# linyueqian/HippoMM

Hardware: AMD Instinct MI355X
Metric: frame-embeddings/sec (ImageBind-huge ViT-H/14 vision tower; scan GB/s under 'scan') (higher is better)
Workload: dtype bf16; 1 GPU; BASELINE cfg2: ViT-H/14 vision encoder (32 blocks, 257 tokens, D=1280), 256 synthetic 224x224 frames per GPU per step (scenes of 6 frames), random-init weights; step = encode -> (N>1: RCCL all-gather of embeddings) -> cosine key-frame selection; frames_per_gpu=256, kept_key_frames=9, of_frames=256

## Files before the change

### hippomm_amd/_lib.py

```python
from __future__ import annotations

import ctypes as C
from pathlib import Path

_PKG = Path(__file__).resolve().parent
LIB_PATH = _PKG / "libhippomm_hip.so"

_lib = None

c_f32p = C.c_void_p
c_ptr = C.c_void_p

_SIGNATURES = {
    "hmm_abi_version": (C.c_int, []),
    "hmm_last_error": (C.c_char_p, []),
    "hmm_device_supported": (C.c_int, []),
    "hmm_cosine_topk_workspace_bytes": (C.c_size_t, [C.c_int64, C.c_int]),
    "hmm_cosine_topk": (C.c_int, [c_ptr, C.c_int64, C.c_int, c_ptr, C.c_int, c_ptr, c_ptr, c_ptr,
                                  c_ptr, C.c_size_t, c_ptr]),
    "hmm_cosine_topk_keys": (C.c_int, [c_ptr, C.c_int64, C.c_int, c_ptr, C.c_int, c_ptr,
                                       c_ptr, C.c_size_t, c_ptr]),
    "hmm_topk_merge_keys": (C.c_int, [c_ptr, C.c_int, C.c_int, c_ptr, c_ptr, c_ptr, c_ptr, c_ptr]),
    "hmm_shadow_store_bytes": (C.c_size_t, [C.c_int64]),
    "hmm_shadow_store_build": (C.c_int, [c_ptr, C.c_int64, C.c_int, c_ptr, C.c_size_t, c_ptr]),
# ... 67 lines not shown
    "hmm_jpeg_workspace_bytes": (C.c_size_t, [c_ptr, C.c_int, C.c_int, C.c_int, C.c_int, C.c_int]),
    "hmm_jpeg_reconstruct": (C.c_int, [c_ptr, C.c_int, C.c_size_t, c_ptr, C.c_int, C.c_int, C.c_int, C.c_int, c_ptr, c_ptr,
                                       C.c_size_t, c_ptr]),
    "hmm_jpeg_entropy_slot_bytes": (C.c_int64, [C.c_size_t]),
    "hmm_jpeg_prepare_entropy": (C.c_int, [c_ptr, C.c_size_t, c_ptr, c_ptr, C.c_size_t]),
    "hmm_jpeg_entropy_workspace_bytes": (C.c_size_t, [c_ptr, C.c_int, C.c_size_t]),
    "hmm_jpeg_decode_coefs_device": (C.c_int, [c_ptr, C.c_int, C.c_size_t, c_ptr, C.c_int, C.c_int, C.c_int, C.c_int, c_ptr,
                                               C.c_size_t, c_ptr, c_ptr, C.c_size_t, c_ptr]),
    "hmm_jpeg_encode_header": (C.c_int, [c_ptr, C.c_int, c_ptr, C.c_size_t, c_ptr]),
    "hmm_jpeg_encode_workspace_bytes": (C.c_size_t, [c_ptr, C.c_int]),
    "hmm_jpeg_encode_bound": (C.c_size_t, [c_ptr]),
    "hmm_jpeg_encode": (C.c_int, [c_ptr, C.c_int, c_ptr, C.c_int, C.c_int, c_ptr, c_ptr, C.c_size_t, c_ptr, C.c_size_t, c_ptr,
                                  c_ptr, C.c_size_t, c_ptr]),
    "hmm_jpeg_encoded_pixels_workspace_bytes": (C.c_size_t, [c_ptr, C.c_int, C.c_int, C.c_int, C.c_int, C.c_int]),
    "hmm_jpeg_encoded_pixels": (C.c_int, [c_ptr, C.c_int, c_ptr, c_ptr, C.c_int, C.c_int, C.c_int, C.c_int, c_ptr, c_ptr,
                                          C.c_size_t, c_ptr]),
    "hmm_encoder_create":(C.c_int, [C.POINTER(C.c_void_p), C.c_int, C.c_int]),
    "hmm_encoder_destroy": (None, [c_ptr]),
    "hmm_encoder_load_param": (C.c_int, [c_ptr, C.c_char_p, c_ptr, C.c_int64, c_ptr]),
    "hmm_encoder_missing_params": (C.c_int, [c_ptr]),
    "hmm_encoder_workspace_bytes": (C.c_size_t, [c_ptr, C.c_int]),
    "hmm_encoder_forward": (C.c_int, [c_ptr, c_ptr, C.c_int, c_ptr, c_ptr, C.c_size_t, c_ptr]),
    "hmm_encoder_flops": (C.c_double, [c_ptr, C.c_int]),
    "hmm_encoder_flops_executed": (C.c_double, [c_ptr, C.c_int]),
    "hmm_encoder_set_streams": (C.c_int, [c_ptr, C.c_int]),
    "hmm_encoder_set_fused_attention": (C.c_int, [c_ptr, C.c_int]),
    "hmm_encoder_text_packed_workspace_bytes": (C.c_size_t, [c_ptr, C.c_int, C.c_int64]),
    "hmm_encoder_forward_text_packed": (C.c_int, [c_ptr, c_ptr, c_ptr, c_ptr, C.c_int, c_ptr, c_ptr, C.c_size_t, c_ptr]),
    "hmm_op_attention_causal_packed_bf16": (C.c_int, [c_ptr, c_ptr, c_ptr, C.c_int, C.c_int, C.c_int, C.c_int, c_ptr]),
    "hmm_op_gemm_bf16": (C.c_int, [c_ptr, c_ptr, c_ptr, c_ptr, C.c_int, C.c_int, C.c_int, C.c_int, c_ptr]),
    "hmm_op_layernorm_bf16": (C.c_int, [c_ptr, c_ptr, c_ptr, c_ptr, C.c_int, C.c_int, C.c_float, c_ptr]),
    "hmm_op_gemm_bf16_tile": (C.c_int, [c_ptr, c_ptr, c_ptr, c_ptr, C.c_int, C.c_int, C.c_int, C.c_int, C.c_int, c_ptr]),
    "hmm_op_gemm_bf16_splitk": (C.c_int, [c_ptr, c_ptr, c_ptr, C.c_int, C.c_int, C.c_int, C.c_int, C.c_int, c_ptr]),
    "hmm_op_gemm_plan": (C.c_int, [C.c_int, C.c_int, C.c_int, C.c_int, C.c_int, C.c_int, C.c_int, c_ptr, C.c_int]),
    "hmm_op_layernorm_reduce_bf16": (C.c_int, [c_ptr, c_ptr, C.c_int, c_ptr, c_ptr, c_ptr, c_ptr, C.c_int, C.c_int, C.c_float, c_ptr]),
    "hmm_op_attention_bf16": (C.c_int, [c_ptr, c_ptr, C.c_int, C.c_int, C.c_int, C.c_int, c_ptr, c_ptr, c_ptr]),
    "hmm_op_qkv_attention_bf16": (C.c_int, [c_ptr, c_ptr, c_ptr, c_ptr, c_ptr, C.c_int, c_ptr]),
    "hmm_op_qkv_attention_audio_bf16": (C.c_int, [c_ptr, c_ptr, c_ptr, c_ptr, c_ptr, c_ptr, C.c_int, c_ptr]),
    "hmm_op_attention_causal_bf16": (C.c_int, [c_ptr, c_ptr, C.c_int, C.c_int, C.c_int, C.c_int, c_ptr]),
    "hmm_op_im2col_vision_bf16": (C.c_int, [c_ptr, c_ptr, C.c_int, c_ptr]),
    "hmm_op_im2col_audio_bf16": (C.c_int, [c_ptr, c_ptr, C.c_int, c_ptr]),
    "hmm_op_fold_conv3d_bf16": (C.c_int, [c_ptr, c_ptr, C.c_int, c_ptr]),
    "hmm_op_assemble_tokens": (C.c_int, [c_ptr, c_ptr, c_ptr, c_ptr, c_ptr, C.c_float, c_ptr, c_ptr, C.c_float, c_ptr,
                                         C.c_int, C.c_int, C.c_int, c_ptr]),
    "hmm_op_layernorm_strided_bf16": (C.c_int, [c_ptr, C.c_size_t, c_ptr, c_ptr, c_ptr, C.c_int, C.c_int, C.c_float, c_ptr]),
    "hmm_op_gather_rows": (C.c_int, [c_ptr, C.c_size_t, c_ptr, C.c_int, C.c_int, c_ptr]),
    "hmm_op_attention_cls_bf16": (C.c_int, [c_ptr, c_ptr, c_ptr, C.c_int, C.c_int, C.c_int, C.c_int, c_ptr, c_ptr, c_ptr]),
    "hmm_op_embed_tokens": (C.c_int, [c_ptr, c_ptr, c_ptr, c_ptr, C.c_int, C.c_int, C.c_int, c_ptr]),
    "hmm_op_layernorm_eos_bf16": (C.c_int, [c_ptr, c_ptr, C.c_int, c_ptr, c_ptr, c_ptr, C.c_int, C.c_int, C.c_float, c_ptr]),
    "hmm_op_l2norm_rows": (C.c_int, [c_ptr, c_ptr, C.c_int, C.c_int, c_ptr, c_ptr]),
    "hmm_op_scan_topk_only": (C.c_int, [c_ptr, C.c_int64, c_ptr, C.c_int, c_ptr, c_ptr]),
    "hmm_op_scan_sims": (C.c_int, [c_ptr, C.c_int64, c_ptr, c_ptr, c_ptr]),
    "hmm_json_find_matrices": (C.c_int, [C.c_char_p, C.c_size_t, C.c_size_t, c_ptr, C.c_int, C.POINTER(C.c_int)]),
    "hmm_json_parse_matrix_f32": (C.c_int, [C.c_char_p, C.c_size_t, C.c_size_t, C.c_size_t, C.c_size_t, c_ptr]),
    "hmm_json_matrix_text_bound": (C.c_size_t, [C.c_size_t, C.c_size_t, C.c_int]),
    "hmm_json_write_matrix_f64": (C.c_int, [c_ptr, C.c_size_t, C.c_size_t, C.c_int, c_ptr, C.c_size_t, C.POINTER(C.c_size_t)]),
    "hmm_json_write_matrix_device_workspace_bytes": (C.c_size_t, [C.c_size_t, C.c_size_t]),
    "hmm_json_write_matrix_device": (C.c_int, [c_ptr, C.c_int, C.c_size_t, C.c_size_t, C.c_int, c_ptr, C.c_size_t, c_ptr, c_ptr,
                                               C.c_size_t, c_ptr]),
    "hmm_json_float_repr": (C.c_int, [c_ptr, C.c_size_t, c_ptr, c_ptr]),
    "hmm_json_parse_matrix_device_workspace_bytes": (C.c_size_t, [C.c_size_t]),
    "hmm_json_parse_matrix_device": (C.c_int, [c_ptr, C.c_size_t, C.c_size_t, C.c_size_t, C.c_size_t, C.c_int, c_ptr, c_ptr, c_ptr,
                                               C.c_int64, c_ptr, C.c_size_t, c_ptr]),
    "hmm_json_float_parse": (C.c_int, [c_ptr, c_ptr, C.c_size_t, c_ptr, c_ptr, c_ptr]),
    "hmm_json_find_matrices_device_workspace_bytes": (C.c_size_t, [C.c_size_t]),
    "hmm_json_find_matrices_device": (C.c_int, [c_ptr, C.c_size_t, C.c_size_t, c_ptr, C.c_int, c_ptr, c_ptr, C.c_size_t, c_ptr]),
    "hmm_json_find_matrices_blocks": (C.c_int, [c_ptr, C.c_size_t, C.c_size_t, c_ptr, C.c_int, c_ptr]),
    "hmm_base64_encoded_length": (C.c_size_t, [C.c_size_t]),
    "hmm_base64_encode_device": (C.c_int, [c_ptr, C.c_int, C.c_size_t, c_ptr, C.c_size_t, c_ptr]),
    "hmm_base64_decode_device": (C.c_int, [c_ptr, C.c_size_t, C.c_int, c_ptr, C.c_size_t, c_ptr, c_ptr]),
    "hmm_base64_encode_host": (C.c_int, [c_ptr, C.c_int, C.c_size_t, c_ptr, C.c_size_t]),
# ... 54 lines not shown
```

### hippomm_amd/csrc/gemm_bf16.hip

```cpp
#include <string>
#include <type_traits>
#include "hmm_common.h"
#include "encoder_ops.h"
#include "gemm_pp_mainloop.h"

namespace hmm {

__device__ __forceinline__ float gelu_erf(float x) {
    const float u = fabsf(x);
    const float t = __builtin_amdgcn_rcpf(fmaf(0.3275911f * 0.70710678118654752440f, u, 1.0f));
    float poly = fmaf(t, 0.5f * 1.061405429f, 0.5f * -1.453152027f);
    poly = fmaf(poly, t, 0.5f * 1.421413741f);
    poly = fmaf(poly, t, 0.5f * -0.284496736f);
    poly = fmaf(poly, t, 0.5f * 0.254829592f);
    poly *= t;
    const float e = __builtin_amdgcn_exp2f(u * u * (-0.5f * 1.4426950408889634f));
    return fmaxf(x, 0.0f) - u * poly * e;
}

template <int EPI, int MI, int NI>
__device__ __forceinline__ void gemm_epilogue(f32x4 (&acc)[MI][NI], const float* __restrict__ bias,
                                              void* __restrict__ Cout, int M, int N, int m_lane, int n_lane) {
    float4 bv[NI];
#pragma unroll
    for (int ni = 0; ni < NI; ++ni)
        bv[ni] = bias ? *reinterpret_cast<const float4*>(bias + n_lane + ni * 16) : make_float4(0.f, 0.f, 0.f, 0.f);

    if constexpr (EPI == HMM_EPI_BIAS_RESID_F32) {
        float* C = static_cast<float*>(Cout);
        float4 xin[2][NI];
        auto load_row = [&](int mi, float4 (&dst)[NI]) {
            const int m = m_lane + mi * 16;
            if (m < M) {
#pragma unroll
                for (int ni = 0; ni < NI; ++ni)
                    dst[ni] = *reinterpret_cast<const float4*>(C + (size_t)m * N + n_lane + ni * 16);
            }
// ... 352 lines not shown
            }
        };
        auto slab_free = [&]() {
            asm volatile("s_waitcnt lgkmcnt(0)" ::: "memory");
            __builtin_amdgcn_wave_barrier();
        };
        if constexpr (RESID) { load_resid(0, 0); load_resid(0, 1); }
        park(0);
        drain(0);
        drain(1);
        slab_free();
        park(1);
        drain(2);
        drain(3);
    }
}

template <int EPI>
__device__ __forceinline__ void gemm_epilogue_lds(f32x4 (&acc)[8][4], const float* __restrict__ bias,
                                                  void* __restrict__ Cout, int M, int N, int m_wave, int n_wave,
                                                  char* slab, int lane) {
    const int fq = lane >> 4;
    float4 bv[4];
#pragma unroll
    for (int ni = 0; ni < 4; ++ni)
        bv[ni] = bias ? *reinterpret_cast<const float4*>(bias + n_wave + ni * 16 + 4 * fq) : make_float4(0.f, 0.f, 0.f, 0.f);
    if (m_wave + 128 <= M)
        gemm_epilogue_lds_body<EPI, false>(acc, bv, Cout, M, N, m_wave, n_wave, slab, lane);
    else if (m_wave < M)
        gemm_epilogue_lds_body<EPI, true>(acc, bv, Cout, M, N, m_wave, n_wave, slab, lane);
}

HMM_TUNABLE(int, g_gemm_walk, -1)
static int pick_walk(int tiles_m, int tiles_n) {
    if (g_gemm_walk >= 0) return g_gemm_walk;
    return (tiles_n >= 10 && tiles_n % 5 == 0 && tiles_m >= 48) ? ((6 << 8) | 5) : 0;
}

template <int EPI>
__global__ __launch_bounds__(512) void gemm_bf16_pp_kernel(
    const bf16_t* __restrict__ A, const bf16_t* __restrict__ W, const float* __restrict__ bias,
    void* __restrict__ Cout, int M, int N, int K, int tiles_n, int walk) {
    extern __shared__ __attribute__((aligned(16))) char smem[];

    const int lane = threadIdx.x & 63;
    const int wave = __builtin_amdgcn_readfirstlane(threadIdx.x >> 6);
    const int wm = wave >> 2, wn = wave & 3;

    const int nb = gridDim.x, bid = blockIdx.x;
    const int q8 = nb >> 3, r8 = nb & 7, xcd = bid & 7;
    const int swz = (xcd < r8 ? xcd * (q8 + 1) : r8 * (q8 + 1) + (xcd - r8) * q8) + (bid >> 3);
    int m0 = (swz / tiles_n) * 256, n0 = (swz % tiles_n) * 256;
    if (walk) {
        const int R = walk >> 8, C = walk & 255, tiles_m = nb / tiles_n;
        const int rg = swz / (R * tiles_n), rem = swz - rg * R * tiles_n;
        const int rows_g = tiles_m - R * rg < R ? tiles_m - R * rg : R;
        const int cg = rem / (rows_g * C), rem2 = rem - cg * rows_g * C;
        const int wc = tiles_n - C * cg < C ? tiles_n - C * cg : C;
        m0 = (rg * R + rem2 / wc) * 256;
        n0 = (cg * C + rem2 % wc) * 256;
    }

    PPSources src;
#pragma unroll
    for (int j = 0; j < 2; ++j) {
        const int lr = (wave + 8 * j) * 8 + (lane >> 3);
        const int c = (lane & 7) ^ ((lr >> 1) & 7);
        const int arow = (lr & 63) + (lr >> 6) * 128;
        int g0 = m0 + arow, g1 = m0 + arow + 64;
        g0 = g0 < M ? g0 : M - 1;
        g1 = g1 < M ? g1 : M - 1;
        src.alo[j] = g0 * K + c * 8;
        src.ahi[j] = g1 * K + c * 8;
        const int bcol = (lr >> 5) * 64 + (lr & 31);
        src.blo[j] = (n0 + bcol) * K + c * 8;
        src.bhi[j] = (n0 + bcol + 32) * K + c * 8;
    }

    f32x4 acc[8][4];
#pragma unroll
    for (int mi = 0; mi < 8; ++mi)
#pragma unroll
        for (int ni = 0; ni < 4; ++ni) acc[mi][ni] = f32x4{0.f, 0.f, 0.f, 0.f};

    pp_mainloop(A, W, src, K >> 6, smem, lane, wave, acc);

    int lane_e = lane;
    asm volatile("" : "+v"(lane_e));
    gemm_epilogue_lds<EPI>(acc, bias, Cout, M, N, m0 + wm * 128, n0 + wn * 64, smem + wave * kEpiSlab, lane_e);
}

template <int EPI>
static int launch_gemm_pp(const bf16_t* A, const bf16_t* W, const float* bias, void* C, int M, int N, int K,
                          hipStream_t st) {
    constexpr int LDS = 8 * kEpiSlab > 2 * 4 * 16384 ? 8 * kEpiSlab : 2 * 4 * 16384;
    const int tiles_m = (M + 255) / 256, tiles_n = N / 256;
    auto kern = gemm_bf16_pp_kernel<EPI>;
    HMM_ENSURE_DYN_LDS(kern, LDS);
    kern<<<tiles_m * tiles_n, 512, LDS, st>>>(A, W, bias, C, M, N, K, tiles_n, pick_walk(tiles_m, tiles_n));
    HMM_LAUNCH_CHECK();
    return HMM_OK;
}

template <int BM, int BN, int WM, int WN, int EPI, int STAGES, int KSUB>
static int launch_gemm(const bf16_t* A, const bf16_t* W, const float* bias, void* C, int M, int N, int K, int splits,
                       hipStream_t st) {
    constexpr int LDS = STAGES * KSUB * (BM + BN) * 128;
    static_assert(LDS <= 160 * 1024, "ring of the tiled GEMM: LDS");
    auto kern = gemm_bf16_kernel<BM, BN, WM, WN, EPI, STAGES, KSUB>;
    HMM_ENSURE_DYN_LDS(kern, LDS);
    const int tiles_m = (M + BM - 1) / BM, tiles_n = N / BN;
    kern<<<tiles_m * tiles_n * splits, WM * WN * 64, LDS, st>>>(A, W, bias, C, M, N, K, tiles_n, tiles_m, K / splits);
    HMM_LAUNCH_CHECK();
    return HMM_OK;
}

struct DispatchRule { const char* knob; int limit; int off; const char* what; const char* forwards; const char* evidence; };
constexpr DispatchRule kDispatchRules[] = {
    {"g_gemm_small_64", 512, 0, "launches of at most this many 64x64 tiles run on them behind the 4-deep ring (else 128x128 ring / double buffer)",
     "text:1,4;vision:1,2;audio:1", "r3_sliver_probe.json, r3_text_latency.json"},
    {"g_gemm_small_32", 400, 0, "launches of at most this many 32x32 tiles run on them (one 16x16 block per wave)",
     "text:1,2;vision:1", "r3_text_latency.json"},
    {"g_gemm_deepk", 1, 0, "deep-K rings: 2 / 4 K-tiles per stage while most CUs have a workgroup of their own (32x32: <= 192 / 256 tiles, 64x64: <= 256)",
     "text:1,2;vision:1", "r4_deepk_probe.json"},
    {"g_gemm_ring8", 1, 0, "the 128-row ring tiles (128x128, 128x64) with eight waves instead of four",
     "vision:1,8;audio:1;text:9", "r5_rect_tile_probe2.json, r5_ring8_ab.json"},
    {"g_gemm_rect", 1, 0, "128x64 ring tiles when 64x64 tiles outnumber the CUs but 128x64 tiles do not, up to g_gemm_rect_rows rows",
     "vision:1;text:4,6;audio:1", "r5_rect_tile_probe.json, r5_rect_forward2.json"},
    {"g_gemm_rect_rows", 700, 320, "row limit of the 128x64 rule (320 = the four-wave tile's)",
     "text:5,6,7,8;audio:1", "r5_rect700_ab.json"},
    {"g_gemm_rect_rows_longk", 1536, 0, "the 128x64 rule's row limit for K >= 5120 (fc2 of three to five frames)",
     "vision:3,4,5", "r5_rect_longk_ab.json"},
// ... 267 lines not shown
    HMM_REQUIRE(M >= 1 && N >= 128 && N % 128 == 0 && splits >= 1 && splits <= 8 && K % (64 * splits) == 0, HMM_E_INVALID,
                "gemm_splitk: unsupported shape M=%d N=%d K=%d splits=%d", M, N, K, splits);
    if (tile < 0) {
        const long w64 = (long)((M + 63) / 64) * (N / 64) * splits;
        const bool k2 = (K / splits) % 128 == 0;
        if (w64 <= 128) tile = k2 ? HMM_GEMM_TILE_32x32_RING_K2 : HMM_GEMM_TILE_32x32_RING;
        else if (w64 <= 256) tile = k2 ? HMM_GEMM_TILE_64x64_RING_K2 : HMM_GEMM_TILE_64x64_RING;
        else if (w64 > 448 && (long)((M + 127) / 128) * (N / 64) * splits <= kNumCU) tile = HMM_GEMM_TILE_128x64_RING;
        else if (w64 > 640) tile = HMM_GEMM_TILE_128x128_RING8;
        else tile = HMM_GEMM_TILE_64x64_RING;
    }
    HMM_REQUIRE(tile >= HMM_GEMM_TILE_128x128_RING && tile <= HMM_GEMM_TILE_64x128_RING8, HMM_E_INVALID,
                "gemm_splitk: tile geometry %d has no split-K launch", tile);
    return plan_push(p, tile, 0, M, N, K, HMM_EPI_F32, splits, 0);
}

int gemm_bf16_splitk(const bf16_t* A, const bf16_t* W, float* part, int M, int N, int K, int splits, int tile, hipStream_t st) {
    HMM_REQUIRE(A && W && part, HMM_E_INVALID, "gemm_splitk: null pointer");
    GemmPlan p;
    const int rc = plan_splitk(p, M, N, K, splits, tile);
    return rc != HMM_OK ? rc : launch_plan(p, A, W, nullptr, part, N, K, HMM_EPI_F32, st);
}

}

using namespace hmm;

extern "C" int hmm_op_gemm_bf16_splitk(const uint16_t* a_dev, const uint16_t* w_dev, float* part_dev, int M, int N, int K,
                                       int splits, int tile, hmm_stream_t stream) {
    return gemm_bf16_splitk(reinterpret_cast<const bf16_t*>(a_dev), reinterpret_cast<const bf16_t*>(w_dev), part_dev, M, N, K,
                            splits, tile, static_cast<hipStream_t>(stream));
}

extern "C" int hmm_op_gemm_plan(int M, int N, int K, int epilogue, int tile, int small_tiles, int splits, int32_t* out, int cap) {
    GemmPlan p;
    HMM_REQUIRE(splits >= 0 && (out || cap <= 0), HMM_E_INVALID, "gemm_plan: splits = %d, out = %p, cap = %d", splits, (void*)out, cap);
    const int rc = splits == 0 ? plan_gemm(p, M, N, K, epilogue, tile, small_tiles) : plan_splitk(p, M, N, K, splits, tile);
    if (rc != HMM_OK) return rc;
    for (int i = 0; i < p.n && i < cap; ++i) {
        const GemmLaunch& l = p.launch[i];
        const int32_t rec[HMM_GEMM_PLAN_FIELDS] = {l.tile, l.row0, l.rows, l.splits, l.sliver_mt, l.flags};
        for (int f = 0; f < HMM_GEMM_PLAN_FIELDS; ++f) out[i * HMM_GEMM_PLAN_FIELDS + f] = rec[f];
    }
    return p.n;
}

extern "C" int hmm_op_gemm_bf16(const uint16_t* a_dev, const uint16_t* w_dev, const float* bias_dev, void* c_dev,
                                int M, int N, int K, int epilogue, hmm_stream_t stream) {
    return gemm_bf16(reinterpret_cast<const bf16_t*>(a_dev), reinterpret_cast<const bf16_t*>(w_dev), bias_dev, c_dev,
                     M, N, K, epilogue, HMM_GEMM_TILE_AUTO, kGemmSmallTiles, static_cast<hipStream_t>(stream));
}

extern "C" int hmm_op_gemm_bf16_tile(const uint16_t* a_dev, const uint16_t* w_dev, const float* bias_dev,
                                     void* c_dev, int M, int N, int K, int epilogue, int tile, hmm_stream_t stream) {
    return gemm_bf16(reinterpret_cast<const bf16_t*>(a_dev), reinterpret_cast<const bf16_t*>(w_dev), bias_dev, c_dev,
                     M, N, K, epilogue, tile, kGemmSmallTiles, static_cast<hipStream_t>(stream));
}
```

### hippomm_amd/csrc/qkv_attention.hip

```cpp
#include "hmm_common.h"
#include "encoder_ops.h"
#include "gemm_pp_mainloop.h"
#include "attention_core.h"

namespace hmm {

struct VisionGeo { static constexpr int D = 1280, H = 16, DH = 80, T = 257, NKT = 9, ROW0 = 1, TAIL = 1; static constexpr bool CLS_OUTSIDE = true, BIAS_KV = false; };
struct AudioGeo  { static constexpr int D = 768,  H = 12, DH = 64, T = 229, NKT = 8, ROW0 = 0, TAIL = 2; static constexpr bool CLS_OUTSIDE = false, BIAS_KV = true; };

template <class G>
struct FusedPlan {
    using Cfg = AttnCfg<G::DH, G::NKT>;
    static constexpr int QRow = G::DH * 2 + 16;
    static constexpr int QOff = Cfg::K_BYTES + Cfg::V_BYTES;
    static constexpr int XOff = QOff + ((G::T * QRow + 15) / 16) * 16;
    static constexpr int Used = XOff + Cfg::X_BYTES;
    static constexpr int Lds = Used > 2 * kPPTile ? Used : 2 * kPPTile;
    static_assert(Lds <= 160 * 1024, "LDS plan of the fused kernel");
    static_assert(G::T + (G::BIAS_KV ? 1 : 0) <= Cfg::NKEY && G::T - G::ROW0 <= 256 && 3 * G::DH <= 256, "tile geometry");
};

#ifdef HMM_PROBE
unsigned long long* g_fused_stamps = nullptr;
extern "C" void hmm_probe_set_fused_stamps(unsigned long long* p) { g_fused_stamps = p; }
#define HMM_FUSED_PROBE_ARG , unsigned long long* stamps
#define HMM_FUSED_PROBE_VAL , g_fused_stamps
#define HMM_FSTAMP(slot, expr) if (stamps && threadIdx.x == 0) stamps[(size_t)blockIdx.x * 16 + (slot)] = (expr);
#else
#define HMM_FUSED_PROBE_ARG
#define HMM_FUSED_PROBE_VAL
#define HMM_FSTAMP(slot, expr)
#endif

template <class G>
__global__ __launch_bounds__(512) void qkv_attention_kernel(
    const bf16_t* __restrict__ a , const bf16_t* __restrict__ w ,
    const float* __restrict__ bias , const bf16_t* __restrict__ qkv_cls ,
    bf16_t* __restrict__ out , int n_img, float scale_log2e,
    const float* __restrict__ bias_k , const float* __restrict__ bias_v, int even_map HMM_FUSED_PROBE_ARG) {
    using P = FusedPlan<G>;
    using Cfg = typename P::Cfg;
    constexpr int kD = G::D, kH = G::H, kDH = G::DH, kT = G::T;
    extern __shared__ __attribute__((aligned(16))) char smem[];
    const int tid = threadIdx.x, lane = tid & 63;
    const int wave = __builtin_amdgcn_readfirstlane(tid >> 6);
    const int wm = wave >> 2, wn = wave & 3;
    const int nb = gridDim.x, q8 = nb >> 3, r8 = nb & 7, xcd = blockIdx.x & 7;
    const int pair = (xcd < r8 ? xcd * (q8 + 1) : r8 * (q8 + 1) + (xcd - r8) * q8) + (blockIdx.x >> 3);
    int b_lin = pair / kH;
    int h = pair % kH;
    if (!even_map) {
        const int n = blockIdx.x >> 3;
        b_lin = (blockIdx.x & 7) + 8 * (n / kH);
        h = n % kH;
        if (b_lin >= n_img) return;
    }
    const int b = n_img - 1 - b_lin;
    HMM_FSTAMP(0, __builtin_amdgcn_s_memrealtime())
    HMM_FSTAMP(6, __builtin_amdgcn_s_memtime())
    HMM_FSTAMP(9, __builtin_amdgcn_s_getreg((20) | (0 << 6) | (31 << 11)))

    PPSources src;
#pragma unroll
    for (int j = 0; j < 2; ++j) {
        const int lr = (wave + 8 * j) * 8 + (lane >> 3);
        const int c = (lane & 7) ^ ((lr >> 1) & 7);
        const int arow = (lr & 63) + (lr >> 6) * 128;
        auto tok_row = [&](int r) {
            const int t = G::ROW0 + r;
            return b * kT + (t < kT ? t : kT - 1);
        };
        src.alo[j] = tok_row(arow) * kD + c * 8;
        src.ahi[j] = tok_row(arow + 64) * kD + c * 8;
        const int bcol = (lr >> 5) * 64 + (lr & 31);
        auto wrow = [&](int col) {
            const int part = col / kDH, d = col - part * kDH;
            return part < 3 ? part * kD + h * kDH + d : h * kDH;
        };
        src.blo[j] = wrow(bcol) * kD + c * 8;
        src.bhi[j] = wrow(bcol + 32) * kD + c * 8;
    }
// ... 50 lines not shown
            const int row = idx / CPR, c = idx - row * CPR;
            *reinterpret_cast<uint4*>(k_lds + row * Cfg::KROW + c * 16) = make_uint4(0u, 0u, 0u, 0u);
            *reinterpret_cast<uint4*>(v_lds + row * Cfg::VROW + c * 16) = make_uint4(0u, 0u, 0u, 0u);
        }
    }
    __syncthreads();
    HMM_FSTAMP(2, __builtin_amdgcn_s_memrealtime())

    const int r = lane & 31, hh = lane >> 5;
    auto load_q = [&](int row, int ks) {
        return *reinterpret_cast<const bf16x8*>(q_lds + row * P::QRow + hh * 16 + ks * 32);
    };
    bf16x8 qf[Cfg::KS];
    {
        const int qrow = wave * 32 + r;
        const int qr = qrow < kT ? qrow : kT - 1;
#pragma unroll
        for (int ks = 0; ks < Cfg::KS; ++ks) qf[ks] = load_q(qr, ks);
    }
    attention_core<kDH, G::NKT>(k_lds, v_lds, reinterpret_cast<float*>(smem + P::XOff), load_q, qf,
                                out + (size_t)b * kT * kD + h * kDH, kT, kT + (G::BIAS_KV ? 1 : 0), kD, scale_log2e, false
#ifdef HMM_PROBE
                                , 0, 1, stamps ? stamps + (size_t)blockIdx.x * 16 : nullptr
#endif
                                );
#ifdef HMM_PROBE
    if (stamps) { asm volatile("s_waitcnt vmcnt(0)" ::: "memory"); __syncthreads(); }
#endif
    HMM_FSTAMP(4, __builtin_amdgcn_s_memrealtime())
    HMM_FSTAMP(8, __builtin_amdgcn_s_memtime())
}

HMM_TUNABLE(int, g_fused_even_map, 1)
template <class G>
static int launch_fused(const bf16_t* a, const bf16_t* w, const float* bias, const bf16_t* qkv_cls, bf16_t* out, int n_img,
                        hipStream_t st, const float* bias_k, const float* bias_v) {
    HMM_REQUIRE(n_img >= 1 && (int64_t)n_img * G::T * G::D < (1ll << 31), HMM_E_INVALID, "qkv_attention: n_img=%d out of range", n_img);
    const float scale_log2e = 1.4426950408889634f / sqrtf((float)G::DH);
    const int grid = g_fused_even_map ? n_img * G::H : 8 * ((n_img + 7) / 8) * G::H;
    auto kern = qkv_attention_kernel<G>;
    HMM_ENSURE_DYN_LDS(kern, FusedPlan<G>::Lds);
    kern<<<grid, 512, FusedPlan<G>::Lds, st>>>(a, w, bias, qkv_cls, out, n_img, scale_log2e, bias_k, bias_v, g_fused_even_map HMM_FUSED_PROBE_VAL);
    HMM_LAUNCH_CHECK();
    return HMM_OK;
}

int qkv_attention_bf16(const bf16_t* a, const bf16_t* w, const float* bias, const bf16_t* qkv_cls, bf16_t* out,
                       int n_img, hipStream_t st) {
    HMM_REQUIRE(a && w && bias && qkv_cls && out, HMM_E_INVALID, "qkv_attention: null pointer");
    return launch_fused<VisionGeo>(a, w, bias, qkv_cls, out, n_img, st, nullptr, nullptr);
}

int qkv_attention_audio_bf16(const bf16_t* a, const bf16_t* w, const float* bias, const float* bias_k, const float* bias_v,
                             bf16_t* out, int n_clips, hipStream_t st) {
    HMM_REQUIRE(a && w && bias && bias_k && bias_v && out, HMM_E_INVALID, "qkv_attention_audio: null pointer");
    return launch_fused<AudioGeo>(a, w, bias, nullptr, out, n_clips, st, bias_k, bias_v);
}

}

using namespace hmm;

extern "C" int hmm_op_qkv_attention_bf16(const uint16_t* a_dev, const uint16_t* w_dev, const float* bias_dev,
                                         const uint16_t* qkv_cls_dev, uint16_t* out_dev, int n_img, hmm_stream_t stream) {
    return qkv_attention_bf16(reinterpret_cast<const bf16_t*>(a_dev), reinterpret_cast<const bf16_t*>(w_dev), bias_dev,
                              reinterpret_cast<const bf16_t*>(qkv_cls_dev), reinterpret_cast<bf16_t*>(out_dev), n_img,
                              static_cast<hipStream_t>(stream));
}

extern "C" int hmm_op_qkv_attention_audio_bf16(const uint16_t* a_dev, const uint16_t* w_dev, const float* bias_dev,
                                               const float* bias_k_dev, const float* bias_v_dev, uint16_t* out_dev,
                                               int n_clips, hmm_stream_t stream) {
    return qkv_attention_audio_bf16(reinterpret_cast<const bf16_t*>(a_dev), reinterpret_cast<const bf16_t*>(w_dev), bias_dev,
                                    bias_k_dev, bias_v_dev, reinterpret_cast<bf16_t*>(out_dev), n_clips,
                                    static_cast<hipStream_t>(stream));
}
```

### include/hippomm_hip.h

```cpp
#ifndef HIPPOMM_HIP_H
#define HIPPOMM_HIP_H

#include <stddef.h>
#include <stdint.h>

#ifdef __cplusplus
extern "C" {
#endif

#define HMM_OK            0
#define HMM_E_INVALID    -1
#define HMM_E_WORKSPACE  -2
#define HMM_E_HIP        -3
#define HMM_E_STATE      -4

#define HMM_FEATURE_DIM  1024

typedef void* hmm_stream_t;


int         hmm_abi_version(void);
const char* hmm_last_error(void);
int         hmm_device_supported(void);

// ... 267 lines not shown
size_t  hmm_jpeg_encoded_pixels_workspace_bytes(const int32_t* geometry, int n, int x0, int y0, int w, int h);
int     hmm_jpeg_encoded_pixels(const void* encode_workspace_dev, int n, const int32_t* geometry, const uint16_t* qtables_dev,
                                int x0, int y0, int w, int h, uint8_t* rgb_out_dev, void* workspace_dev, size_t workspace_bytes,
                                hmm_stream_t stream);

#define HMM_EPI_BIAS_BF16        0
#define HMM_EPI_BIAS_GELU_BF16   1
#define HMM_EPI_BIAS_RESID_F32   2
#define HMM_EPI_F32              3

int hmm_op_gemm_bf16(const uint16_t* a_dev, const uint16_t* w_dev, const float* bias_dev,
                     void* c_dev, int M, int N, int K, int epilogue, hmm_stream_t stream);
#define HMM_GEMM_TILE_AUTO       -1
#define HMM_GEMM_TILE_AUTO_TILED -2
#define HMM_GEMM_TILE_128x128     0
#define HMM_GEMM_TILE_256x128     1
#define HMM_GEMM_TILE_256x256     2
#define HMM_GEMM_TILE_256x256_PP  3
#define HMM_GEMM_TILE_PP_PEELED   4
#define HMM_GEMM_TILE_SLIVER      5
#define HMM_GEMM_TILE_128x128_RING 6
#define HMM_GEMM_TILE_64x64_RING  7
#define HMM_GEMM_TILE_32x32_RING  8
#define HMM_GEMM_TILE_32x32_RING_K2 9
#define HMM_GEMM_TILE_64x64_RING_K2 11
#define HMM_GEMM_TILE_128x64_RING 12
#define HMM_GEMM_TILE_64x128_RING 13
#define HMM_GEMM_TILE_128x128_RING8 14
#define HMM_GEMM_TILE_128x64_RING8  15
#define HMM_GEMM_TILE_64x128_RING8  16
#define HMM_GEMM_TILE_32x32_RING_K4 10
int hmm_op_gemm_bf16_tile(const uint16_t* a_dev, const uint16_t* w_dev, const float* bias_dev,
                          void* c_dev, int M, int N, int K, int epilogue, int tile, hmm_stream_t stream);
int hmm_op_gemm_bf16_splitk(const uint16_t* a_dev, const uint16_t* w_dev, float* part_dev, int M, int N, int K,
                            int splits, int tile, hmm_stream_t stream);
#define HMM_GEMM_PLAN_FIELDS       6
#define HMM_GEMM_PLAN_PP_TAIL      1
#define HMM_GEMM_PLAN_SLIVER_PEEL  2
int hmm_op_gemm_plan(int M, int N, int K, int epilogue, int tile, int small_tiles, int splits, int32_t* out, int cap);
int hmm_op_layernorm_reduce_bf16(float* x_dev, const float* part_dev, int splits, const float* bias_dev,
                                 const float* gamma_dev, const float* beta_dev, uint16_t* y_dev, int rows, int D,
                                 float eps, hmm_stream_t stream);
int hmm_op_layernorm_bf16(const float* x_dev, const float* gamma_dev, const float* beta_dev,
                          uint16_t* y_dev, int rows, int D, float eps, hmm_stream_t stream);
int hmm_op_attention_bf16(const uint16_t* qkv_dev, uint16_t* out_dev, int batch, int tokens,
                          int heads, int head_dim, const float* bias_k_dev, const float* bias_v_dev,
                          hmm_stream_t stream);
int hmm_op_qkv_attention_bf16(const uint16_t* a_dev, const uint16_t* w_dev, const float* bias_dev,
                              const uint16_t* qkv_cls_dev, uint16_t* out_dev, int n_img, hmm_stream_t stream);
int hmm_op_qkv_attention_audio_bf16(const uint16_t* a_dev, const uint16_t* w_dev, const float* bias_dev,
                                    const float* bias_k_dev, const float* bias_v_dev, uint16_t* out_dev, int n_clips,
                                    hmm_stream_t stream);
int hmm_op_attention_causal_bf16(const uint16_t* qkv_dev, uint16_t* out_dev, int batch, int tokens,
                                 int heads, int head_dim, hmm_stream_t stream);
int hmm_op_attention_causal_packed_bf16(const uint16_t* qkv_dev, uint16_t* out_dev, const int32_t* offsets_dev, int batch,
                                        int total_rows, int heads, int head_dim, hmm_stream_t stream);

int hmm_op_im2col_vision_bf16(const float* frames_dev, uint16_t* out_dev, int n_img, hmm_stream_t stream);
int hmm_op_im2col_audio_bf16(const float* mels_dev, uint16_t* out_dev, int n_clip, hmm_stream_t stream);
int hmm_op_fold_conv3d_bf16(const float* w_dev, uint16_t* dst_dev, int D, hmm_stream_t stream);
int hmm_op_assemble_tokens(const float* patches_dev, const float* cls_dev, const float* pos_dev,
                           const float* stem_gamma_dev, const float* stem_beta_dev, float stem_eps,
                           const float* pre_gamma_dev, const float* pre_beta_dev, float pre_eps,
                           float* x_dev, int n_img, int T, int D, hmm_stream_t stream);
int hmm_op_layernorm_strided_bf16(const float* x_dev, size_t in_stride, const float* gamma_dev, const float* beta_dev,
                                  uint16_t* y_dev, int rows, int D, float eps, hmm_stream_t stream);
int hmm_op_gather_rows(const void* src_dev, size_t src_row_stride_bytes, void* dst_dev, int n_rows, int row_bytes,
                       hmm_stream_t stream);
int hmm_op_attention_cls_bf16(const uint16_t* q_cls_dev, const uint16_t* kv_dev, uint16_t* out_dev, int batch, int tokens,
                              int heads, int head_dim, const float* bias_k_dev, const float* bias_v_dev,
                              hmm_stream_t stream);
int hmm_op_embed_tokens(const int64_t* ids_dev, const float* table_dev, const float* pos_dev, float* x_dev, int n_rows,
                        int T, int vocab, hmm_stream_t stream);
int hmm_op_layernorm_eos_bf16(const float* x_dev, const int64_t* ids_dev, int T, const float* gamma_dev,
                              const float* beta_dev, uint16_t* y_dev, int batch, int D, float eps, hmm_stream_t stream);
int hmm_op_l2norm_rows(const float* v_dev, float* out_dev, int n_out, int clips, const float* log_scale_dev,
                       hmm_stream_t stream);

int hmm_op_scan_topk_only(const float* store_dev, int64_t n_rows, const float* query_dev, int k,
                          uint64_t* cand_keys_dev, hmm_stream_t stream);
int hmm_op_scan_sims(const float* store_dev, int64_t n_rows, const float* query_dev, float* sims_dev,
                     hmm_stream_t stream);

typedef struct hmm_json_matrix { size_t begin, end, rows, cols; } hmm_json_matrix;
int hmm_json_find_matrices(const char* text, size_t len, size_t min_values, hmm_json_matrix* out, int cap, int* n_found);
// ... 74 lines not shown
```

Measured before the change: 3295 frame-embeddings/s.

## Reorder GEMM tile walk and group attention heads per XCD for L2 reuse

Moves the XCD-aware block-to-tile mapping into a shared header and adds a column-outer walk (8 row tiles by 4 column groups) that the ping-pong GEMM picks by default when tiles_n is divisible by 4. The fused QKV-attention kernel now deals blocks so that consecutive blocks on an XCD share a group of heads across images (default group 4 for vision), aiming to keep weight panels resident in L2. It also exposes host entry points to launch with an explicit walk or group and to inspect the mapping. A different walk can lower L2 hit rates for some shapes and change load balance across XCDs.

After: 3319 frame-embeddings/s, median of 6. About the same (+0.7%).

```diff
diff --git a/hippomm_amd/_lib.py b/hippomm_amd/_lib.py
--- a/hippomm_amd/_lib.py
+++ b/hippomm_amd/_lib.py
@@ -123,11 +123,14 @@
     "hmm_op_layernorm_bf16": (C.c_int, [c_ptr, c_ptr, c_ptr, c_ptr, C.c_int, C.c_int, C.c_float, c_ptr]),
     "hmm_op_gemm_bf16_tile": (C.c_int, [c_ptr, c_ptr, c_ptr, c_ptr, C.c_int, C.c_int, C.c_int, C.c_int, C.c_int, c_ptr]),
     "hmm_op_gemm_bf16_splitk": (C.c_int, [c_ptr, c_ptr, c_ptr, C.c_int, C.c_int, C.c_int, C.c_int, C.c_int, c_ptr]),
+    "hmm_op_gemm_bf16_walk": (C.c_int, [c_ptr, c_ptr, c_ptr, c_ptr, C.c_int, C.c_int, C.c_int, C.c_int, C.c_int, c_ptr]),
+    "hmm_op_panel_deal": (C.c_int, [C.c_int, C.c_int, C.c_int, C.c_int, c_ptr, C.c_int]),
     "hmm_op_gemm_plan": (C.c_int, [C.c_int, C.c_int, C.c_int, C.c_int, C.c_int, C.c_int, C.c_int, c_ptr, C.c_int]),
     "hmm_op_layernorm_reduce_bf16": (C.c_int, [c_ptr, c_ptr, C.c_int, c_ptr, c_ptr, c_ptr, c_ptr, C.c_int, C.c_int, C.c_float, c_ptr]),
     "hmm_op_attention_bf16": (C.c_int, [c_ptr, c_ptr, C.c_int, C.c_int, C.c_int, C.c_int, c_ptr, c_ptr, c_ptr]),
     "hmm_op_qkv_attention_bf16": (C.c_int, [c_ptr, c_ptr, c_ptr, c_ptr, c_ptr, C.c_int, c_ptr]),
     "hmm_op_qkv_attention_audio_bf16": (C.c_int, [c_ptr, c_ptr, c_ptr, c_ptr, c_ptr, c_ptr, C.c_int, c_ptr]),
+    "hmm_op_qkv_attention_group_bf16": (C.c_int, [C.c_int, c_ptr, c_ptr, c_ptr, c_ptr, c_ptr, c_ptr, c_ptr, C.c_int, C.c_int, c_ptr]),
     "hmm_op_attention_causal_bf16": (C.c_int, [c_ptr, c_ptr, C.c_int, C.c_int, C.c_int, C.c_int, c_ptr]),
     "hmm_op_im2col_vision_bf16": (C.c_int, [c_ptr, c_ptr, C.c_int, c_ptr]),
     "hmm_op_im2col_audio_bf16": (C.c_int, [c_ptr, c_ptr, C.c_int, c_ptr]),
diff --git a/hippomm_amd/csrc/gemm_bf16.hip b/hippomm_amd/csrc/gemm_bf16.hip
--- a/hippomm_amd/csrc/gemm_bf16.hip
+++ b/hippomm_amd/csrc/gemm_bf16.hip
@@ -3,6 +3,7 @@
 #include "hmm_common.h"
 #include "encoder_ops.h"
 #include "gemm_pp_mainloop.h"
+#include "panel_deal.h"
 
 namespace hmm {
 
@@ -421,9 +422,11 @@
 }
 
 HMM_TUNABLE(int, g_gemm_walk, -1)
+static_assert(kWalkColOuter == HMM_GEMM_WALK_COL_OUTER, "walk encoding of the public header");
 static int pick_walk(int tiles_m, int tiles_n) {
     if (g_gemm_walk >= 0) return g_gemm_walk;
-    return (tiles_n >= 10 && tiles_n % 5 == 0 && tiles_m >= 48) ? ((6 << 8) | 5) : 0;
+    if (!(tiles_n >= 10 && tiles_n % 5 == 0 && tiles_m >= 48)) return 0;
+    return tiles_n % 4 == 0 && g_gemm_walk != -2 ? (kWalkColOuter | (8 << 8) | 4) : ((6 << 8) | 5);
 }
 
 template <int EPI>
@@ -436,19 +439,8 @@
     const int wave = __builtin_amdgcn_readfirstlane(threadIdx.x >> 6);
     const int wm = wave >> 2, wn = wave & 3;
 
-    const int nb = gridDim.x, bid = blockIdx.x;
-    const int q8 = nb >> 3, r8 = nb & 7, xcd = bid & 7;
-    const int swz = (xcd < r8 ? xcd * (q8 + 1) : r8 * (q8 + 1) + (xcd - r8) * q8) + (bid >> 3);
-    int m0 = (swz / tiles_n) * 256, n0 = (swz % tiles_n) * 256;
-    if (walk) {
-        const int R = walk >> 8, C = walk & 255, tiles_m = nb / tiles_n;
-        const int rg = swz / (R * tiles_n), rem = swz - rg * R * tiles_n;
-        const int rows_g = tiles_m - R * rg < R ? tiles_m - R * rg : R;
-        const int cg = rem / (rows_g * C), rem2 = rem - cg * rows_g * C;
-        const int wc = tiles_n - C * cg < C ? tiles_n - C * cg : C;
-        m0 = (rg * R + rem2 / wc) * 256;
-        n0 = (cg * C + rem2 % wc) * 256;
-    }
+    const int tile = gemm_walk_tile(xcd_run_pos(gridDim.x, blockIdx.x), gridDim.x / tiles_n, tiles_n, walk);
+    const int m0 = (tile / tiles_n) * 256, n0 = (tile % tiles_n) * 256;
 
     PPSources src;
 #pragma unroll
@@ -481,12 +473,12 @@
 
 template <int EPI>
 static int launch_gemm_pp(const bf16_t* A, const bf16_t* W, const float* bias, void* C, int M, int N, int K,
-                          hipStream_t st) {
+                          hipStream_t st, int walk = -1 ) {
     constexpr int LDS = 8 * kEpiSlab > 2 * 4 * 16384 ? 8 * kEpiSlab : 2 * 4 * 16384;
     const int tiles_m = (M + 255) / 256, tiles_n = N / 256;
     auto kern = gemm_bf16_pp_kernel<EPI>;
     HMM_ENSURE_DYN_LDS(kern, LDS);
-    kern<<<tiles_m * tiles_n, 512, LDS, st>>>(A, W, bias, C, M, N, K, tiles_n, pick_walk(tiles_m, tiles_n));
+    kern<<<tiles_m * tiles_n, 512, LDS, st>>>(A, W, bias, C, M, N, K, tiles_n, walk < 0 ? pick_walk(tiles_m, tiles_n) : walk);
     HMM_LAUNCH_CHECK();
     return HMM_OK;
 }
@@ -820,6 +812,28 @@
                             splits, tile, static_cast<hipStream_t>(stream));
 }
 
+extern "C" int hmm_op_gemm_bf16_walk(const uint16_t* a_dev, const uint16_t* w_dev, const float* bias_dev, void* c_dev,
+                                     int M, int N, int K, int epilogue, int walk, hmm_stream_t stream) {
+    HMM_REQUIRE(a_dev && w_dev && c_dev && (epilogue == HMM_EPI_F32 || bias_dev), HMM_E_INVALID, "gemm_walk: null pointer");
+    HMM_REQUIRE(M >= 1 && N >= 256 && N % 256 == 0 && K >= 128 && K % 128 == 0 && pp_offsets_fit(M, N, K), HMM_E_INVALID,
+                "gemm_walk: unsupported shape M=%d N=%d K=%d (the ping-pong kernel: N%%256==0, K%%128==0)", M, N, K);
+    HMM_REQUIRE(walk >= 0 && (walk & ~(kWalkColOuter | 0xffff)) == 0 && (walk == 0 || ((walk & 255) && ((walk >> 8) & 255))),
+                HMM_E_INVALID, "gemm_walk: walk = %d", walk);
+    return dispatch_epi(epilogue, [&](auto epi_c) {
+        return launch_gemm_pp<decltype(epi_c)::value>(reinterpret_cast<const bf16_t*>(a_dev), reinterpret_cast<const bf16_t*>(w_dev),
+                                                      bias_dev, c_dev, M, N, K, static_cast<hipStream_t>(stream), walk);
+    });
+}
+
+extern "C" int hmm_op_panel_deal(int kind, int a, int b, int setting, int32_t* items_out, int cap) {
+    HMM_REQUIRE((kind == 0 || kind == 1) && a >= 1 && b >= 1 && (int64_t)a * b < (1 << 24) && items_out && cap >= a * b, HMM_E_INVALID,
+                "panel_deal: kind = %d, %d x %d, cap = %d", kind, a, b, cap);
+    const int nb = a * b;
+    for (int bid = 0; bid < nb; ++bid)
+        items_out[bid] = kind == 0 ? fused_deal(xcd_run_pos(nb, bid), a, b, setting) : gemm_walk_tile(xcd_run_pos(nb, bid), a, b, setting);
+    return nb;
+}
+
 extern "C" int hmm_op_gemm_plan(int M, int N, int K, int epilogue, int tile, int small_tiles, int splits, int32_t* out, int cap) {
     GemmPlan p;
     HMM_REQUIRE(splits >= 0 && (out || cap <= 0), HMM_E_INVALID, "gemm_plan: splits = %d, out = %p, cap = %d", splits, (void*)out, cap);
diff --git a/hippomm_amd/csrc/panel_deal.h b/hippomm_amd/csrc/panel_deal.h
--- /dev/null
+++ b/hippomm_amd/csrc/panel_deal.h
@@ -0,0 +1,46 @@
+#pragma once
+
+namespace hmm {
+
+#if defined(__HIPCC__) || defined(__CUDACC__)
+#define HMM_HD __host__ __device__
+#else
+#define HMM_HD
+#endif
+
+HMM_HD inline int xcd_run_pos(int nb, int bid) {
+    const int q8 = nb >> 3, r8 = nb & 7, xcd = bid & 7;
+    return (xcd < r8 ? xcd * (q8 + 1) : r8 * (q8 + 1) + (xcd - r8) * q8) + (bid >> 3);
+}
+
+HMM_HD inline int fused_deal(int pos, int n_img, int heads, int group) {
+    if (group <= 0 || group >= heads || n_img * group < 32) return pos;
+    const int hg = pos / (n_img * group);
+    const int gs = heads - hg * group < group ? heads - hg * group : group;
+    const int rem = pos - hg * n_img * group;
+    return (rem / gs) * heads + hg * group + rem % gs;
+}
+
+constexpr int kWalkColOuter = 1 << 16;
+HMM_HD inline int gemm_walk_tile(int pos, int tiles_m, int tiles_n, int walk) {
+    const int R = (walk >> 8) & 255, C = walk & 255;
+    if (R == 0 || C == 0) return pos;
+    int rg, cg, rem;
+    if (walk & kWalkColOuter) {
+        cg = pos / (tiles_m * C);
+        const int wc = tiles_n - C * cg < C ? tiles_n - C * cg : C;
+        rem = pos - cg * tiles_m * C;
+        rg = rem / (R * wc);
+        rem -= rg * R * wc;
+    } else {
+        rg = pos / (R * tiles_n);
+        rem = pos - rg * R * tiles_n;
+        const int rows_g = tiles_m - R * rg < R ? tiles_m - R * rg : R;
+        cg = rem / (rows_g * C);
+        rem -= cg * rows_g * C;
+    }
+    const int wc = tiles_n - C * cg < C ? tiles_n - C * cg : C;
+    return (rg * R + rem / wc) * tiles_n + cg * C + rem % wc;
+}
+
+}
diff --git a/hippomm_amd/csrc/qkv_attention.hip b/hippomm_amd/csrc/qkv_attention.hip
--- a/hippomm_amd/csrc/qkv_attention.hip
+++ b/hippomm_amd/csrc/qkv_attention.hip
@@ -2,11 +2,12 @@
 #include "encoder_ops.h"
 #include "gemm_pp_mainloop.h"
 #include "attention_core.h"
+#include "panel_deal.h"
 
 namespace hmm {
 
-struct VisionGeo { static constexpr int D = 1280, H = 16, DH = 80, T = 257, NKT = 9, ROW0 = 1, TAIL = 1; static constexpr bool CLS_OUTSIDE = true, BIAS_KV = false; };
-struct AudioGeo  { static constexpr int D = 768,  H = 12, DH = 64, T = 229, NKT = 8, ROW0 = 0, TAIL = 2; static constexpr bool CLS_OUTSIDE = false, BIAS_KV = true; };
+struct VisionGeo { static constexpr int D = 1280, H = 16, DH = 80, T = 257, NKT = 9, ROW0 = 1, TAIL = 1, GROUP = 4; static constexpr bool CLS_OUTSIDE = true, BIAS_KV = false; };
+struct AudioGeo  { static constexpr int D = 768,  H = 12, DH = 64, T = 229, NKT = 8, ROW0 = 0, TAIL = 2, GROUP = 12; static constexpr bool CLS_OUTSIDE = false, BIAS_KV = true; };
 
 template <class G>
 struct FusedPlan {
@@ -37,7 +38,7 @@
     const bf16_t* __restrict__ a , const bf16_t* __restrict__ w ,
     const float* __restrict__ bias , const bf16_t* __restrict__ qkv_cls ,
     bf16_t* __restrict__ out , int n_img, float scale_log2e,
-    const float* __restrict__ bias_k , const float* __restrict__ bias_v, int even_map HMM_FUSED_PROBE_ARG) {
+    const float* __restrict__ bias_k , const float* __restrict__ bias_v, int even_map, int group HMM_FUSED_PROBE_ARG) {
     using P = FusedPlan<G>;
     using Cfg = typename P::Cfg;
     constexpr int kD = G::D, kH = G::H, kDH = G::DH, kT = G::T;
@@ -45,8 +46,7 @@
     const int tid = threadIdx.x, lane = tid & 63;
     const int wave = __builtin_amdgcn_readfirstlane(tid >> 6);
     const int wm = wave >> 2, wn = wave & 3;
-    const int nb = gridDim.x, q8 = nb >> 3, r8 = nb & 7, xcd = blockIdx.x & 7;
-    const int pair = (xcd < r8 ? xcd * (q8 + 1) : r8 * (q8 + 1) + (xcd - r8) * q8) + (blockIdx.x >> 3);
+    const int pair = fused_deal(xcd_run_pos(gridDim.x, blockIdx.x), n_img, kH, group);
     int b_lin = pair / kH;
     int h = pair % kH;
     if (!even_map) {
@@ -163,15 +163,17 @@
 }
 
 HMM_TUNABLE(int, g_fused_even_map, 1)
+HMM_TUNABLE(int, g_fused_head_group, 0)
 template <class G>
 static int launch_fused(const bf16_t* a, const bf16_t* w, const float* bias, const bf16_t* qkv_cls, bf16_t* out, int n_img,
-                        hipStream_t st, const float* bias_k, const float* bias_v) {
+                        hipStream_t st, const float* bias_k, const float* bias_v, int group = 0 ) {
+    if (group <= 0) group = g_fused_head_group > 0 ? g_fused_head_group : G::GROUP;
     HMM_REQUIRE(n_img >= 1 && (int64_t)n_img * G::T * G::D < (1ll << 31), HMM_E_INVALID, "qkv_attention: n_img=%d out of range", n_img);
     const float scale_log2e = 1.4426950408889634f / sqrtf((float)G::DH);
     const int grid = g_fused_even_map ? n_img * G::H : 8 * ((n_img + 7) / 8) * G::H;
     auto kern = qkv_attention_kernel<G>;
     HMM_ENSURE_DYN_LDS(kern, FusedPlan<G>::Lds);
-    kern<<<grid, 512, FusedPlan<G>::Lds, st>>>(a, w, bias, qkv_cls, out, n_img, scale_log2e, bias_k, bias_v, g_fused_even_map HMM_FUSED_PROBE_VAL);
+    kern<<<grid, 512, FusedPlan<G>::Lds, st>>>(a, w, bias, qkv_cls, out, n_img, scale_log2e, bias_k, bias_v, g_fused_even_map, group HMM_FUSED_PROBE_VAL);
     HMM_LAUNCH_CHECK();
     return HMM_OK;
 }
@@ -197,6 +199,20 @@
     return qkv_attention_bf16(reinterpret_cast<const bf16_t*>(a_dev), reinterpret_cast<const bf16_t*>(w_dev), bias_dev,
                               reinterpret_cast<const bf16_t*>(qkv_cls_dev), reinterpret_cast<bf16_t*>(out_dev), n_img,
                               static_cast<hipStream_t>(stream));
+}
+
+extern "C" int hmm_op_qkv_attention_group_bf16(int audio, const uint16_t* a_dev, const uint16_t* w_dev, const float* bias_dev,
+                                               const uint16_t* qkv_cls_dev, const float* bias_k_dev, const float* bias_v_dev,
+                                               uint16_t* out_dev, int n, int head_group, hmm_stream_t stream) {
+    HMM_REQUIRE(a_dev && w_dev && bias_dev && out_dev && (audio ? bias_k_dev && bias_v_dev : qkv_cls_dev != nullptr), HMM_E_INVALID,
+                "qkv_attention_group: null pointer");
+    HMM_REQUIRE(head_group >= 1, HMM_E_INVALID, "qkv_attention_group: head_group = %d", head_group);
+    const bf16_t* a = reinterpret_cast<const bf16_t*>(a_dev);
+    const bf16_t* w = reinterpret_cast<const bf16_t*>(w_dev);
+    bf16_t* out = reinterpret_cast<bf16_t*>(out_dev);
+    hipStream_t st = static_cast<hipStream_t>(stream);
+    if (audio) return launch_fused<AudioGeo>(a, w, bias_dev, nullptr, out, n, st, bias_k_dev, bias_v_dev, head_group);
+    return launch_fused<VisionGeo>(a, w, bias_dev, reinterpret_cast<const bf16_t*>(qkv_cls_dev), out, n, st, nullptr, nullptr, head_group);
 }
 
 extern "C" int hmm_op_qkv_attention_audio_bf16(const uint16_t* a_dev, const uint16_t* w_dev, const float* bias_dev,
diff --git a/include/hippomm_hip.h b/include/hippomm_hip.h
--- a/include/hippomm_hip.h
+++ b/include/hippomm_hip.h
@@ -323,6 +323,10 @@
 #define HMM_GEMM_TILE_32x32_RING_K4 10
 int hmm_op_gemm_bf16_tile(const uint16_t* a_dev, const uint16_t* w_dev, const float* bias_dev,
                           void* c_dev, int M, int N, int K, int epilogue, int tile, hmm_stream_t stream);
+#define HMM_GEMM_WALK_COL_OUTER (1 << 16)
+int hmm_op_gemm_bf16_walk(const uint16_t* a_dev, const uint16_t* w_dev, const float* bias_dev,
+                          void* c_dev, int M, int N, int K, int epilogue, int walk, hmm_stream_t stream);
+int hmm_op_panel_deal(int kind, int a, int b, int setting, int32_t* items_out, int cap);
 int hmm_op_gemm_bf16_splitk(const uint16_t* a_dev, const uint16_t* w_dev, float* part_dev, int M, int N, int K,
                             int splits, int tile, hmm_stream_t stream);
 #define HMM_GEMM_PLAN_FIELDS       6
@@ -342,6 +346,9 @@
 int hmm_op_qkv_attention_audio_bf16(const uint16_t* a_dev, const uint16_t* w_dev, const float* bias_dev,
                                     const float* bias_k_dev, const float* bias_v_dev, uint16_t* out_dev, int n_clips,
                                     hmm_stream_t stream);
+int hmm_op_qkv_attention_group_bf16(int audio, const uint16_t* a_dev, const uint16_t* w_dev, const float* bias_dev,
+                                    const uint16_t* qkv_cls_dev, const float* bias_k_dev, const float* bias_v_dev,
+                                    uint16_t* out_dev, int n, int head_group, hmm_stream_t stream);
 int hmm_op_attention_causal_bf16(const uint16_t* qkv_dev, uint16_t* out_dev, int batch, int tokens,
                                  int heads, int head_dim, hmm_stream_t stream);
 int hmm_op_attention_causal_packed_bf16(const uint16_t* qkv_dev, uint16_t* out_dev, const int32_t* offsets_dev, int batch,
```
